# falcon-xu/DeViT

Hardware: AMD Instinct MI355X
Metric: images/sec distill_sub step (DeiT-B->dedeit, bs256, 224^2) (higher is better)
Workload: dtype bf16; 1 GPU; distill_sub step dedeit<-deit_base_distilled_patch16_224, num_division=4 (C=25), bs=256/GPU, 224x224, hard distillation, drop_path 0.1, AdamW+EMA; classes=25, global_batch=256, parallelism=dp1

## Files before the change

devit_amd/_lib.py:

```python
import ctypes as C
import os

import torch

_HERE = os.path.dirname(os.path.abspath(__file__))
LIB_PATH = os.environ.get("DEVIT_LIB_PATH") or os.path.join(_HERE, "libdevit_hip.so")

EPI_STORE_BF16, EPI_GELU_BF16, EPI_RESIDUAL_F32, EPI_PATCH_F32, EPI_DGELU_BF16, EPI_ATOMIC_F32, EPI_STORE_F32 = range(7)


class Epilogue(C.Structure):
    _fields_ = [("kind", C.c_int), ("out", C.c_void_p), ("ldc", C.c_int), ("bias", C.c_void_p),
                ("colscale", C.c_void_p), ("aux", C.c_void_p), ("aux_in", C.c_void_p), ("res", C.c_void_p),
                ("rowscale", C.c_void_p), ("rows_per_scale", C.c_int), ("pos", C.c_void_p),
                ("patch_tokens", C.c_int), ("extra_tokens", C.c_int), ("exact_gelu", C.c_int),
                ("out_batch_stride", C.c_longlong), ("m_valid", C.c_int), ("dtype16", C.c_int)]


class Operand(C.Structure):
    _fields_ = [("ptr", C.c_void_p), ("ld", C.c_int), ("kmajor", C.c_int), ("row_group", C.c_int),
                ("row_skip", C.c_int), ("batch_stride", C.c_longlong)]


ACT_LN1, ACT_MEAN1, ACT_RSTD1, ACT_QKV, ACT_ATTN_O, ACT_LSE, ACT_X1, ACT_ATT, ACT_LN2, ACT_MEAN2, ACT_RSTD2, ACT_H, ACT_H_PRE, \
    ACT_X2, ACT_COUNT = range(15)
BLK_SAVE, BLK_QKV_PAD, BLK_ATT = 1, 2, 4
BWD_DH_PRE, BWD_DLN2, BWD_DX1, BWD_G1, BWD_DATTN, BWD_DQKV, BWD_DLN1, BWD_LNWS, BWD_COUNT = range(9)


class BlockWeights(C.Structure):
    _fields_ = [(n, C.c_void_p) for n in ("n1w", "n1b", "qkv_b", "proj_b", "n2w", "n2b", "fc1_b", "fc2_b", "qkv_w16",
                                          "proj_w16", "fc1_w16", "fc2_w16", "head_gate", "neuron_gate")] + \
               [("num_heads", C.c_int), ("attn_width", C.c_int), ("hidden", C.c_int), ("dtype16", C.c_int), ("fc2_w16t", C.c_void_p)]


class BlockWgrads(C.Structure):
    _fields_ = [(n, C.c_void_p) for n in ("n1w", "n1b", "qkv_w", "qkv_b", "proj_w", "proj_b", "n2w", "n2b", "fc1_w",
                                          "fc1_b", "fc2_w", "fc2_b")]


class BlockActs(C.Structure):
    _fields_ = [("x", C.c_void_p), ("buf", C.c_void_p * 14), ("dp1", C.c_void_p), ("dp2", C.c_void_p), ("flags", C.c_int)]


class BlockBwdIO(C.Structure):
    _fields_ = [("dx", C.c_void_p), ("g2", C.c_void_p), ("dx_in", C.c_void_p), ("g_prev", C.c_void_p),
                ("prev_dp2", C.c_void_p), ("prev_fc2_b_grad", C.c_void_p), ("g2_bias_done", C.c_int),
                ("dqkv_add", C.c_void_p), ("ws", C.c_void_p * 8), ("lnws_bytes", C.c_size_t),
                ("defer_jobs", C.c_void_p), ("defer_count", C.c_void_p)]


class BlockDropout(C.Structure):
    _fields_ = [("seed", C.c_ulonglong), ("block", C.c_int), ("thr", C.c_uint), ("thr_attn", C.c_uint), ("scale_keep", C.c_float),
                ("scale_keep_attn", C.c_float), ("tmp", C.c_void_p)]


class IndexJob(C.Structure):
    _fields_ = [("src", C.c_void_p), ("dst", C.c_void_p), ("idx", C.c_void_p), ("rows", C.c_int), ("cols", C.c_int),
                ("src_ld", C.c_int), ("dst_ld", C.c_int), ("mode", C.c_int), ("elem", C.c_int)]


class WgradJob(C.Structure):
    _fields_ = [("a", C.c_void_p), ("lda", C.c_int), ("a_cols", C.c_int), ("b", C.c_void_p), ("ldb", C.c_int), ("out", C.c_void_p),
                ("ldc", C.c_int), ("transposed", C.c_int), ("a_colsum", C.c_void_p)]


class MixSample(C.Structure):
    _fields_ = [("mode", C.c_int), ("lam", C.c_float), ("y0", C.c_int), ("y1", C.c_int), ("x0", C.c_int), ("x1", C.c_int),
                ("reserved", C.c_int * 2)]


class OptChunk(C.Structure):
    _fields_ = [("first4", C.c_uint), ("count4", C.c_uint), ("segment", C.c_int), ("flags", C.c_int)]


OPT_CHUNK_GRANULES, OPT_CHUNK_NO_DECAY = 1024, 1

HAS_Y_BF16, HAS_Y_F32, HAS_DY_F32, HAS_DRES, HAS_DX, HAS_DX_BF16, HAS_DQKV_ADD = 1, 2, 4, 8, 16, 32, 64


class LaunchInfo(C.Structure):
    _fields_ = [("name", C.c_char_p)] + [(n, C.c_int) for n in ("a_kmajor", "b_kmajor", "kind", "M", "N", "K", "batch", "split_k", "rows",
                                                                "width", "q_rows", "has", "njobs", "a_cols")] + \
               [("flops", C.c_double), ("bytes", C.c_double)]


LAUNCH_OBSERVER = C.CFUNCTYPE(None, C.c_void_p, C.c_int, C.c_void_p, C.POINTER(LaunchInfo))

HSIC_BF16, HSIC_F16, HSIC_F32 = range(3)

DROP_POS, DROP_ATTN, DROP_PROJ, DROP_HIDDEN, DROP_FC2 = range(5)

ROUTE_TILE128, ROUTE_TILE256, ROUTE_FULL_ROW, ROUTE_GEMM4 = 1, 3, 4, 5

WGRAD_MAX_JOBS = 48
ABI_VERSION = 3
ABI_STRUCTS = {0: Epilogue, 1: Operand, 2: BlockWeights, 3: BlockWgrads, 4: BlockActs, 5: BlockBwdIO, 6: IndexJob, 7: WgradJob, 8: LaunchInfo, 9: BlockDropout,
               10: MixSample, 11: OptChunk}


class DevitError(RuntimeError):
    pass


_P, _I, _F, _Z, _LL = C.c_void_p, C.c_int, C.c_float, C.c_size_t, C.c_longlong
_U64, _U32 = C.c_ulonglong, C.c_uint

SIGNATURES = {
    "devit_version": (_I, []),
    "devit_last_error": (C.c_char_p, []),
    "devit_check_device": (_I, [_I]),
    "devit_abi_struct_size": (_Z, [_I]),
    "devit_set_launch_observer": (_I, [LAUNCH_OBSERVER, _P]),
    "devit_gemm_full_row_selected": (_I, [_I, _I, _I, _I]),
    "devit_wgrad_grouped": (_I, [C.POINTER(WgradJob), _I, _I, _I, _P]),
    "devit_gemm_bf16": (_I, [C.POINTER(Operand), C.POINTER(Operand), _I, _I, _I, _I, _I, C.POINTER(Epilogue), _P]),
    "devit_gemm_route": (_I, [C.POINTER(Operand), C.POINTER(Operand), _I, _I, _I, _I, _I, C.POINTER(Epilogue)]),
    "devit_set_reserved_cus": (_I, [_I]),
    "devit_get_reserved_cus": (_I, []),
    "devit_set_deterministic": (_I, [_I]),
    "devit_get_deterministic": (_I, []),
    "devit_det_workspace_bytes": (_Z, []),
    "devit_set_det_workspace": (_I, [_P, _Z]),
    "devit_layernorm_fwd": (_I, [_P, _I, _I, _I, _I, _P, _P, _F, _P, _P, _P, _P, _I, _P]),
    "devit_layernorm_bwd_workspace": (_Z, [_I, _I]),
    "devit_layernorm_bwd": (_I, [_P, _I, _P, _I, _I, _I, _I, _P, _P, _P, _P, _P, _P, _P, _I, _P, _P, _P, _I, _P, _Z, _P]),
    "devit_dgrad_layernorm_bwd_fused": (_I, [_I, _I, _I]),
    "devit_dgrad_layernorm_bwd": (_I, [_P, _P, _I, _I, _P, _P, _I, _I, _P, _P, _P, _P, _P, _P, _P, _I, _P, _P, _P, _I, _P, _Z, _P]),
    "devit_block_acts_sizes": (_I, [_I, _I, _I, _I, _I, _I, C.POINTER(C.c_size_t)]),
    "devit_block_bwd_sizes": (_I, [_I, _I, _I, _I, _I, C.POINTER(C.c_size_t)]),
    "devit_encoder_fwd": (_I, [_I, C.POINTER(BlockWeights), C.POINTER(BlockActs), _I, _I, _I, _F, _P]),
    "devit_block_bwd": (_I, [C.POINTER(BlockWeights), C.POINTER(BlockActs), C.POINTER(BlockWgrads), C.POINTER(BlockBwdIO),
                             _I, _I, _I, _F, _P]),
    "devit_encoder_fwd_drop": (_I, [_I, C.POINTER(BlockWeights), C.POINTER(BlockActs), C.POINTER(BlockDropout), _I, _I, _I, _F, _P]),
    "devit_block_bwd_drop": (_I, [C.POINTER(BlockWeights), C.POINTER(BlockActs), C.POINTER(BlockWgrads), C.POINTER(BlockBwdIO),
                                  C.POINTER(BlockDropout), _I, _I, _I, _F, _P]),
    "devit_attn_fwd": (_I, [_P, _P, _P, _P, _I, _I, _I, _I, _F, _I, _P]),
    "devit_attn_bwd": (_I, [_P, _P, _P, _P, _P, _P, _P, _I, _I, _I, _I, _F, _P]),
    "devit_attn_fwd_rows": (_I, [_P, _I, _P, _I, _P, _P, _P, _I, _I, _I, _I, _I, _F, _I, _P]),
    "devit_attn_bwd_rows": (_I, [_P, _I, _P, _I, _P, _P, _P, _P, _P, _I, _P, _I, _I, _I, _I, _I, _I, _F, _P]),
    "devit_dropout_mask": (_I, [_U64, _I, _I, _U32, _I, _I, _LL, _P, _P]),
    "devit_dropout_apply": (_I, [_P, _I, _I, _I, _I, _LL, _U64, _I, _I, _U32, _F, _P, _P]),
    "devit_dropout_residual": (_I, [_P, _P, _P, _P, _I, _I, _I, _U64, _I, _I, _U32, _F, _P]),
    "devit_attn_fwd_drop": (_I, [_P, _P, _P, _P, _I, _I, _I, _I, _F, _U64, _I, _U32, _F, _P]),
    "devit_attn_bwd_drop": (_I, [_P, _P, _P, _P, _P, _P, _P, _I, _I, _I, _I, _F, _U64, _I, _U32, _F, _P]),
    "devit_index_copy": (_I, [_P, _I, _I, _P]),
    "devit_hsic_target": (_I, [_P, _I, _I, _I, _P, _P, _Z, _P]),
    "devit_hsic_scores_workspace": (_Z, [_I, _I, _I]),
    "devit_hsic_scores": (_I, [_P, _I, _I, _I, _I, _I, _LL, _LL, _P, _P, _P, _P, _P, _Z, _P]),
    "devit_hsic_head_pairs": (_I, [_P, _I, _I, _P, _P]),
    "devit_im2row_bf16": (_I, [_P, _P, _I, _I, _I, _I, _I, _I, _P]),
    "devit_mix_im2row_bf16": (_I, [_P, _P, _P, _I, _I, C.c_double, _I, _I, _I, _I, _P]),
    "devit_mix_im2row_bf16_sized": (_I, [_P, _P, _P, _I, _I, C.c_double, _I, _I, _I, _I, _I, _I, _P]),
    "devit_mix_targets": (_I, [_P, _P, _I, _I, C.c_double, C.c_double, _P]),
    "devit_mix_im2row_table": (_I, [_P, _P, _P, _P, _P, _I, _P]),
    "devit_mix_im2row_table_sized": (_I, [_P, _P, _P, _P, _P, _I, _I, _I, _P]),
    "devit_mix_targets_table": (_I, [_P, _P, _P, _I, _I, C.c_double, _P]),
    "devit_embed_tokens": (_I, [_P, _P, _P, _P, _I, _I, _I, _P]),
    "devit_embed_bwd": (_I, [_P, _I, _I, _I, _I, _P, _P, _P, _P, _P, _I, _P]),
    "devit_cast_bf16": (_I, [_P, _P, _Z, _I, _P]),
    "devit_scale_cast_bf16": (_I, [_P, _P, _P, _I, _I, _I, _P]),
    "devit_colsum_workspace": (_Z, [_I, _I]),
    "devit_colsum_bf16": (_I, [_P, _I, _I, _I, _I, _I, _P, _I, _P, _Z, _P]),
    "devit_sgemm_small": (_I, [_P, _LL, _LL, _P, _LL, _LL, _P, _P, _I, _I, _I, _I, _F, _I, _P]),
    "devit_sumsq_workspace": (_Z, []),
    "devit_sumsq_f32": (_I, [_P, _Z, _P, _P, _Z, _P]),
    "devit_adamw_step": (_I, [_P, _P, _P, _P, _P, _P, _P, _P, _P, _Z, _F, _F, _F, _F, _F, _F, _F, _P]),
    "devit_sgd_step": (_I, [_P, _P, _P, _P, _P, _P, _P, _P, _Z, _F, _I, _F, _F, _F, _F, _P]),
    "devit_adam_l2_step": (_I, [_P, _P, _P, _P, _P, _P, _P, _P, _P, _Z, _F, _F, _F, _F, _F, _F, _F, _P]),
    "devit_lamb_workspace": (_Z, [_I, _I]),
    "devit_lamb_step": (_I, [_P, _P, _P, _P, _P, _P, _P, _P, _Z, _P, _I, _I, _I, _F, _F, _F, _F, _F, _F, _F, _P, _Z, _P]),
    "devit_cls_distill_loss": (_I, [_P, _P, _P, _P, _I, _I, _I, _F, _F, _P, _P, _P, _P]),
    "devit_token_mse": (_I, [_P, _P, _Z, _P, _P, _I, _P]),
    "devit_token_kldiv": (_I, [_P, _P, _Z, _I, _P, _P, _I, _P]),
    "devit_relation_stats": (_I, [_P, _P, _I, _I, _I, _I, _I, _P, _P, _P, _P, _P]),
    "devit_relation_grad": (_I, [_P, _P, _P, _P, _P, _I, _I, _I, _I, _I, _P, _I, _P]),
    "devit_add_scale_cast_bf16": (_I, [_P, _P, _P, _P, _I, _I, _I, _P]),
    "devit_hid_normalize": (_I, [_P, _P, _P, _I, _I, _I, _I, _I, _I, _F, _P]),
    "devit_hid_stats": (_I, [_P, _P, _I, _I, _I, _I, _P, _P, _P]),
    "devit_hid_grad": (_I, [_P, _P, _P, _I, _I, _I, _I, _P, _I, _P]),
    "devit_hid_normalize_bwd": (_I, [_P, _P, _P, _P, _I, _I, _I, _I, _I, _P]),
    "devit_gemm_f32": (_I, [_P, _LL, _LL, _LL, _LL, _P, _LL, _LL, _LL, _LL, _I, _I, _I, _I, _I, _LL, _LL, _I, _I, _F, _P, _I,
                            C.POINTER(Epilogue), _P]),
    "devit_softmax_rows_f32": (_I, [_P, _I, _I, _I, _F, _P, _P]),
    "devit_softmax_bwd_rows_f32": (_I, [_P, _P, _I, _I, _I, _F, _P]),
    "devit_im2row_f32": (_I, [_P, _P, _I, _P]),
    "devit_im2row_f32_sized": (_I, [_P, _P, _I, _I, _I, _P]),
    "devit_scale_rows_f32": (_I, [_P, _P, _P, _I, _I, _I, _P]),
    "devit_colsum_f32": (_I, [_P, _I, _I, _I, _P, _I, _P]),
    "devit_comm_unique_id": (_I, [_P]),
    "devit_comm_init": (_I, [_P, _I, _I, C.POINTER(C.c_void_p)]),
    "devit_comm_allreduce_f32": (_I, [_P, _P, _Z, _P]),
    "devit_comm_destroy": (_I, [_P]),
}

_lib = None
_checked_devices = set()


def load():
    global _lib
    if _lib is None:
        if not os.path.exists(LIB_PATH):
            raise DevitError(
                f"{LIB_PATH} not found: build it with `python -c 'import __graft_entry__ as g; g.build()'` "
                "(or devit_amd/csrc/build.sh).  devit_amd has no CPU / PyTorch fallback.")
        lib = C.CDLL(LIB_PATH)
        for name, (res, args) in SIGNATURES.items():
            fn = getattr(lib, name)
            fn.restype, fn.argtypes = res, args
        if lib.devit_version() != ABI_VERSION:
            raise DevitError(f"libdevit_hip.so ABI version {lib.devit_version()} != {ABI_VERSION} of this binding: rebuild (devit_amd/csrc/build.sh)")
        for which, cls in ABI_STRUCTS.items():
            if lib.devit_abi_struct_size(which) != C.sizeof(cls):
                raise DevitError(f"libdevit_hip.so: sizeof struct {which} = {lib.devit_abi_struct_size(which)}, the binding's {cls.__name__} has "
                                 f"{C.sizeof(cls)} bytes: header and binding disagree")
        _lib = lib
    return _lib


def require_device(t: torch.Tensor):
    if not t.is_cuda:
        raise DevitError("devit_amd ops run on MI355X (gfx950) only; got a %s tensor. There is no CPU fallback "
                         "(the CPU restatement lives in oracle/ and is test infrastructure)." % t.device)
    idx = t.device.index if t.device.index is not None else torch.cuda.current_device()
    if idx not in _checked_devices:
        call("devit_check_device", idx)
        _checked_devices.add(idx)


before_call = None


def call(name, *args):
    lib = load()
    if before_call is not None:
        before_call()
    rc = getattr(lib, name)(*args)
    if rc != 0:
        raise DevitError(f"{name} failed ({rc}): {lib.devit_last_error().decode()}")
    return rc


def stream_ptr():
    return C.c_void_p(torch.cuda.current_stream().cuda_stream)


def ptr(t):
    return None if t is None else C.c_void_p(t.data_ptr())
```

devit_amd/ops.py:

```python
import contextlib
import ctypes as C
import os

import numpy as np
import torch

from . import _lib as L
from ._lib import ptr, stream_ptr

BF16, F16, F32 = torch.bfloat16, torch.float16, torch.float32
ROW_TILE = 256


PROFILE = None
PROFILE_HBM = None
PROFILE_WGRAD = None


def gemm_template(a_kmajor, b_kmajor, kind, fused_ln_bwd=False):
    b_row = not b_kmajor or kind == L.EPI_RESIDUAL_F32
    return ("A_km" if a_kmajor else "A_row") + "/" + ("B_row" if b_row else "B_km") + ("+ln_bwd" if fused_ln_bwd else "")


def hbm_record(i):
# ... 1058 lines not shown


class HeadsFn(torch.autograd.Function):
    @staticmethod
    def forward(ctx, x, norm_w, norm_b, head_w, head_b, headd_w, headd_b, ntok, eps, grad_ready):
        L.require_device(x)
        x = x.contiguous()
        B, T, D = x.shape
        rows = B * ntok
        dev = x.device
        tok = torch.empty((B, ntok, D), dtype=F32, device=dev)
        mean = torch.empty(rows, dtype=F32, device=dev)
        rstd = torch.empty(rows, dtype=F32, device=dev)
        layernorm_fwd(x.view(B * T, D), rows, D, norm_w, norm_b, eps, y_f32=tok, mean=mean, rstd=rstd, in_group=ntok,
                      in_stride=T)
        outs = [tok]
        if head_w is not None:
            Cn = head_w.shape[0]
            lo = torch.empty((B, Cn), dtype=F32, device=dev)
            sgemm_small(tok, ntok * D, 1, head_w, D, 1, head_b, lo, Cn, B, Cn, D)
            outs.append(lo)
            if ntok == 2 and headd_w is not None:
                lk = torch.empty((B, Cn), dtype=F32, device=dev)
                sgemm_small(tok[:, 1], ntok * D, 1, headd_w, D, 1, headd_b, lk, Cn, B, Cn, D)
                outs.append(lk)
        ctx.save = (x, tok, mean, rstd)
        ctx.params = (norm_w, norm_b, head_w, head_b, headd_w, headd_b)
        ctx.meta = (B, T, D, ntok, eps, grad_ready)
        ctx.set_materialize_grads(False)
        return tuple(outs)

    @staticmethod
    def backward(ctx, dtok, dlo=None, dlk=None):
        x, tok, mean, rstd = ctx.save
        norm_w, norm_b, head_w, head_b, headd_w, headd_b = ctx.params
        B, T, D, ntok, eps, grad_ready = ctx.meta
        dev = x.device
        dt = torch.zeros((B, ntok, D), dtype=F32, device=dev) if dtok is None else dtok.contiguous().clone()
        for j, (dl, w, b) in enumerate(((dlo, head_w, head_b), (dlk, headd_w, headd_b))):
            if dl is None or w is None:
                continue
            dl = dl.contiguous()
            Cn = w.shape[0]
            sgemm_small(dl, Cn, 1, w, 1, D, None, dt[:, j], ntok * D, B, D, Cn, accumulate=True)
            sgemm_small(dl, 1, Cn, tok[:, j], 1, ntok * D, None, grad_buf(w), D, Cn, D, B, accumulate=True)
            ones = _ones1(dev)
            sgemm_small(dl, 1, Cn, ones, 0, 0, None, grad_buf(b), 1, Cn, 1, B, accumulate=True)
        dx = torch.zeros((B, T, D), dtype=F32, device=dev)
        layernorm_bwd(dt, True, x.view(B * T, D), B * ntok, D, mean, rstd, norm_w, None, dx.view(B * T, D), None, None,
                      0, grad_buf(norm_w), grad_buf(norm_b), in_group=ntok, in_stride=T)
        if grad_ready is not None:
            grad_ready([p for p in ctx.params if p is not None])
        return (dx,) + (None,) * 9


def _to_rows_bf16(x):
    B, N, D = x.shape
    M = B * N
    buf = rows_alloc(M, D, BF16, x.device)
    call("devit_scale_cast_bf16", ptr(x.contiguous().float()), ptr(buf), None, 0, M, D, stream_ptr())
    return buf


class MlpFn(torch.autograd.Function):
    @staticmethod
    def forward(ctx, x, module, w1, b1, w2, b2, w1_16, w2_16, gate, grad_enabled):
        L.require_device(x)
        B, N, D = x.shape
        M, dev, Hd, Do = B * N, x.device, w1.shape[0], w2.shape[0]
        xb = _to_rows_bf16(x)
        need = grad_enabled and (x.requires_grad or w1.requires_grad)
        h = rows_alloc(M, Hd, BF16, dev)
        h_pre = rows_alloc(M, Hd, BF16, dev) if need else None
        linear_fwd(xb, w1_16, b1, M, out=h, kind=L.EPI_GELU_BF16, colscale=gate, aux=h_pre, exact_gelu=0)
        y = torch.empty((B, N, Do), dtype=F32, device=dev)
        linear_fwd(h, w2_16, b2, M, out=y.view(M, Do), kind=L.EPI_STORE_F32)
        module.neuron_output = h[:M].view(B, N, Hd)
        ctx.s = (xb, h, h_pre, gate, w1, b1, w2, b2, w1_16, w2_16, (B, N, D))
        return y

    @staticmethod
    def backward(ctx, dy):
        xb, h, h_pre, gate, w1, b1, w2, b2, w1_16, w2_16, (B, N, D) = ctx.s
        M, dev, Hd = B * N, dy.device, w1.shape[0]
        g = _to_rows_bf16(dy)
        dh = rows_alloc(M, Hd, BF16, dev)
        linear_dgrad(g, w2_16, M, out=dh, kind=L.EPI_DGELU_BF16, colscale=gate, aux_in=h_pre)
        linear_wgrad(g, h, grad_buf(w2), grad_buf(b2), M)
        dx = torch.empty((B, N, D), dtype=F32, device=dev)
        linear_dgrad(dh, w1_16, M, out=dx.view(M, D), kind=L.EPI_STORE_F32)
        linear_wgrad(dh, xb, grad_buf(w1), grad_buf(b1), M)
        return (dx,) + (None,) * 9


class AttentionFn(torch.autograd.Function):
    @staticmethod
    def forward(ctx, x, module, wq, bq, wp, bp_, wq16, wp16, gate, grad_enabled):
        L.require_device(x)
        B, N, D = x.shape
        M, dev, H = B * N, x.device, module.num_heads
        xb = _to_rows_bf16(x)
        need = grad_enabled and (x.requires_grad or wq.requires_grad)
        qkv = rows_alloc(M, 3 * D, BF16, dev)
        linear_fwd(xb, wq16, bq, M, out=qkv)
        o = rows_alloc(M, D, BF16, dev)
        lse = torch.empty((B, H, N), dtype=F32, device=dev) if need else None
        call("devit_attn_fwd", ptr(qkv), ptr(o), ptr(lse), ptr(gate), B, N, H, D // H, (D // H) ** -0.5, 0, stream_ptr())
        y = torch.empty((B, N, D), dtype=F32, device=dev)
        linear_fwd(o, wp16, bp_, M, out=y.view(M, D), kind=L.EPI_STORE_F32)
        module.head_output = o[:M].view(B, N, H, D // H)
        ctx.s = (xb, qkv, o, lse, gate, wq, bq, wp, bp_, wq16, wp16, (B, N, D, H))
        return y, qkv

    @staticmethod
    def backward(ctx, dy, dqkv_in):
        xb, qkv, o, lse, gate, wq, bq, wp, bp_, wq16, wp16, (B, N, D, H) = ctx.s
        M, dev = B * N, dy.device
        g = _to_rows_bf16(dy)
        do = rows_alloc(M, D, BF16, dev)
        linear_dgrad(g, wp16, M, out=do)
        linear_wgrad(g, o, grad_buf(wp), grad_buf(bp_), M)
        dqkv = rows_alloc(M, 3 * D, BF16, dev)
        call("devit_attn_bwd", ptr(qkv), ptr(o), ptr(do), ptr(lse), ptr(gate),
             ptr(dqkv_in.contiguous()) if dqkv_in is not None else None, ptr(dqkv), B, N, H, D // H, (D // H) ** -0.5,
             stream_ptr())
        dx = torch.empty((B, N, D), dtype=F32, device=dev)
        linear_dgrad(dqkv, wq16, M, out=dx.view(M, D), kind=L.EPI_STORE_F32)
        linear_wgrad(dqkv, xb, grad_buf(wq), grad_buf(bq), M)
        return (dx,) + (None,) * 9


class ClsDistillLossFn(torch.autograd.Function):

    @staticmethod
    def forward(ctx, logits, logits_kd, teacher_logits, soft_targets, kind, alpha, tau):
        L.require_device(logits)
        logits, logits_kd = logits.contiguous().float(), logits_kd.contiguous().float()
        soft_targets = soft_targets.contiguous().float()
        tl = teacher_logits.contiguous().float() if teacher_logits is not None else None
        B, Cn = logits.shape
        loss3 = torch.empty(3, dtype=F32, device=logits.device)
        dlo, dlk = torch.empty_like(logits), torch.empty_like(logits_kd)
        call("devit_cls_distill_loss", ptr(logits), ptr(logits_kd), ptr(tl), ptr(soft_targets), B, Cn,
             {"none": 0, "soft": 1, "hard": 2}[kind], alpha, tau, ptr(loss3), ptr(dlo), ptr(dlk), stream_ptr())
        ctx.save_for_backward(dlo, dlk)
        return loss3[0]

    @staticmethod
    def backward(ctx, g):
        dlo, dlk = ctx.saved_tensors
        return dlo * g, dlk * g, None, None, None, None, None


class RelationLossFn(torch.autograd.Function):

    @staticmethod
    def forward(ctx, s_qkv, t_qkv, B, N, hd_s, hd_t):
        L.require_device(s_qkv)
        dev = s_qkv.device
        Ds, Dt = s_qkv.shape[1] // 3, t_qkv.shape[1] // 3
        assert s_qkv.shape[0] >= (B - 1) * N + 256 and t_qkv.shape[0] >= (B - 1) * N + 256, "packed qkv needs pad rows"
        losses = torch.empty(3, dtype=F32, device=dev)
        grams, stats = [], []
        for j in range(3):
            gt = torch.empty((B, 256, 256), dtype=F32, device=dev)
            gs = torch.empty((B, 256, 256), dtype=F32, device=dev)
            for buf, Dm, out in ((t_qkv, Dt, gt), (s_qkv, Ds, gs)):
                f = buf[:, j * Dm:]
                gemm(f, 3 * Dm, 0, f, 3 * Dm, 0, 256, 256, Dm, kind=L.EPI_STORE_F32, out=out, ldc=256, batch=B,
                     a_bs=N * 3 * Dm, b_bs=N * 3 * Dm, out_bs=256 * 256, dtype16=int(buf.dtype == F16))
            lse_t = torch.empty((B, N), dtype=F32, device=dev)
            lse_s = torch.empty((B, N), dtype=F32, device=dev)
            row_kl = torch.empty((B, N), dtype=F32, device=dev)
            call("devit_relation_stats", ptr(gt), ptr(gs), B, N, 256, hd_t, hd_s, ptr(lse_t), ptr(lse_s), ptr(row_kl),
                 ptr(losses[j:]), stream_ptr())
            grams.append((gt, gs))
            stats.append((lse_t, lse_s))
        ctx.grams, ctx.stats, ctx.s_qkv = grams, stats, s_qkv
        ctx.meta = (B, N, hd_s, hd_t, Ds)
        return losses

    @staticmethod
    def backward(ctx, g):
        B, N, hd_s, hd_t, Ds = ctx.meta
        s_qkv = ctx.s_qkv
        dev = s_qkv.device
        g = g.contiguous().float()
        d = torch.empty_like(s_qkv)
        S = torch.empty((B, 256, 256), dtype=BF16, device=dev)
        for j in range(3):
            gt, gs = ctx.grams[j]
            lse_t, lse_s = ctx.stats[j]
            call("devit_relation_grad", ptr(gt), ptr(gs), ptr(lse_t), ptr(lse_s), ptr(g[j:]), B, N, 256, hd_t, hd_s,
                 ptr(S), 0, stream_ptr())
            f = s_qkv[:, j * Ds:]
            gemm(S, 256, 0, f, 3 * Ds, 1, 256, Ds, 256, kind=L.EPI_STORE_BF16, out=d[:, j * Ds:], ldc=3 * Ds, batch=B,
                 a_bs=256 * 256, b_bs=N * 3 * Ds, out_bs=N * 3 * Ds, m_valid=N)
        ctx.grams = ctx.stats = None
        return d, None, None, None, None, None


HID_EPS = 1e-12


def hid_normalize(h, exact=False):
    L.require_device(h)
    if h.dim() != 3:
        raise L.DevitError(f"cal_hid_relation_loss: hidden states are [B, N, D], got {tuple(h.shape)}")
    B, N, D = h.shape
    h = h.contiguous().float()
    if h.data_ptr() % 16:
        h = h.clone()
    ld = (D + 127) // 128 * 128
    rows = pad_rows(B * N) + qkv_pad_rows(N)
    hn = torch.empty((rows, ld), dtype=F32 if exact else BF16, device=h.device)
    inv = torch.empty(B * N, dtype=F32, device=h.device)
    call("devit_hid_normalize", ptr(h), ptr(hn), ptr(inv), B, N, D, ld, rows, int(exact), HID_EPS, stream_ptr())
    return hn, inv


def hid_gram(hn, B, N, D, exact=False):
    ld = hn.shape[1]
    if exact:
        from .ops_f32 import sgemm
        g = torch.zeros((B, 256, 256), dtype=F32, device=hn.device)
        sgemm(hn, ld, 1, hn, ld, 1, N, N, D, out=g, ldc=256, batch=B, a_bo=N * ld, b_bo=N * ld, c_bo=65536)
        return g
    g = torch.empty((B, 256, 256), dtype=F32, device=hn.device)
    gemm(hn, ld, 0, hn, ld, 0, 256, 256, ld, kind=L.EPI_STORE_F32, out=g, ldc=256, batch=B, a_bs=N * ld, b_bs=N * ld, out_bs=65536)
    return g


def hid_stats(gs, gt, B, N, layers=1):
    row_sq = torch.empty(B * N, dtype=F32, device=gs.device)
    loss = torch.empty(1, dtype=F32, device=gs.device)
    call("devit_hid_stats", ptr(gs), ptr(gt), B, N, 256, layers, ptr(row_sq), ptr(loss), stream_ptr())
    return loss


def hid_grad(gs, gt, upstream, B, N, layers=1, exact=False):
    S = torch.empty((B, 256, 256), dtype=F32 if exact else BF16, device=gs.device)
    call("devit_hid_grad", ptr(gs), ptr(gt), ptr(upstream), B, N, 256, layers, ptr(S), int(exact), stream_ptr())
    return S


def hid_dhn(S, hn, B, N, D, exact=False):
    ld = hn.shape[1]
    if exact:
        from .ops_f32 import sgemm
        dhn = torch.zeros((B * N, ld), dtype=F32, device=hn.device)
        sgemm(S, 256, 1, hn, 1, ld, N, D, N, out=dhn, ldc=ld, batch=B, a_bo=65536, b_bo=N * ld, c_bo=N * ld)
        return dhn
    dhn = torch.empty((B * N, ld), dtype=F32, device=hn.device)
    gemm(S, 256, 0, hn, ld, 1, 256, ld, 256, kind=L.EPI_STORE_F32, out=dhn, ldc=ld, batch=B, a_bs=65536, b_bs=N * ld, out_bs=N * ld,
         m_valid=N)
    return dhn


def hid_normalize_bwd(hn, dhn, inv, B, N, D):
    dh = torch.empty((B, N, D), dtype=F32, device=hn.device)
    call("devit_hid_normalize_bwd", ptr(hn), ptr(dhn), ptr(inv), ptr(dh), B, N, D, hn.shape[1], int(hn.dtype == F32), stream_ptr())
    return dh


class HidRelationLossFn(torch.autograd.Function):

    @staticmethod
    def forward(ctx, s, t, layers, exact):
        B, N, Ds = s.shape
        if tuple(t.shape[:2]) != (B, N):
            raise L.DevitError(f"cal_hid_relation_loss: student {tuple(s.shape)} and teacher {tuple(t.shape)} differ in batch or tokens")
        hs, inv_s = hid_normalize(s, exact)
        ht, _ = hid_normalize(t, exact)
        gs, gt = hid_gram(hs, B, N, Ds, exact), hid_gram(ht, B, N, t.shape[2], exact)
        ctx.keep, ctx.meta = (hs, inv_s, gs, gt), (B, N, Ds, layers, exact)
        return hid_stats(gs, gt, B, N, layers)[0]

    @staticmethod
    def backward(ctx, g):
        hs, inv_s, gs, gt = ctx.keep
        B, N, Ds, layers, exact = ctx.meta
        ctx.keep = None
        S = hid_grad(gs, gt, g.contiguous().float(), B, N, layers, exact)
        return hid_normalize_bwd(hs, hid_dhn(S, hs, B, N, Ds, exact), inv_s, B, N, Ds), None, None, None
```

include/devit_hip.h:

```cpp
#ifndef DEVIT_HIP_H
#define DEVIT_HIP_H

#include <stddef.h>
#include <stdint.h>

#ifdef __cplusplus
extern "C" {
#endif

#define DEVIT_ABI_VERSION 3
#define DEVIT_API __attribute__((visibility("default")))

enum {
  DEVIT_OK = 0,
  DEVIT_ERR_SHAPE = -1,
  DEVIT_ERR_ARG = -2,
  DEVIT_ERR_LAUNCH = -3,
  DEVIT_ERR_DEVICE = -4
};

DEVIT_API int devit_version(void);
DEVIT_API const char* devit_last_error(void);
DEVIT_API int devit_check_device(int dev);
DEVIT_API size_t devit_abi_struct_size(int which);
// ... 110 lines not shown
                        float scale, unsigned long long seed, int block, unsigned thr, float scale_keep, void* stream);
DEVIT_API int devit_attn_bwd_drop(const void* qkv, const void* out, const void* dout, const float* lse, const float* head_gate,
                        const void* dqkv_add, void* dqkv, int B, int N, int H, int head_dim, float scale, unsigned long long seed,
                        int block, unsigned thr, float scale_keep, void* stream);

typedef struct {
  const float *n1w, *n1b, *qkv_b, *proj_b, *n2w, *n2b, *fc1_b, *fc2_b;
  const void *qkv_w16, *proj_w16, *fc1_w16, *fc2_w16;
  const float *head_gate, *neuron_gate;
  int num_heads, attn_width, hidden;
  int dtype16;
  const void* fc2_w16t;
} devit_block_weights;

typedef struct {
  float *n1w, *n1b, *qkv_w, *qkv_b, *proj_w, *proj_b, *n2w, *n2b, *fc1_w, *fc1_b, *fc2_w, *fc2_b;
} devit_block_wgrads;

enum { DEVIT_ACT_LN1 = 0, DEVIT_ACT_MEAN1, DEVIT_ACT_RSTD1, DEVIT_ACT_QKV, DEVIT_ACT_ATTN_O, DEVIT_ACT_LSE, DEVIT_ACT_X1,
       DEVIT_ACT_ATT, DEVIT_ACT_LN2, DEVIT_ACT_MEAN2, DEVIT_ACT_RSTD2, DEVIT_ACT_H, DEVIT_ACT_H_PRE, DEVIT_ACT_X2,
       DEVIT_ACT_COUNT };
enum { DEVIT_BLK_SAVE = 1, DEVIT_BLK_QKV_PAD = 2, DEVIT_BLK_ATT = 4 };

typedef struct {
  const float* x;
  void* buf[DEVIT_ACT_COUNT];
  const float *dp1, *dp2;
  int flags;
} devit_block_acts;

enum { DEVIT_BWD_DH_PRE = 0, DEVIT_BWD_DLN2, DEVIT_BWD_DX1, DEVIT_BWD_G1, DEVIT_BWD_DATTN, DEVIT_BWD_DQKV, DEVIT_BWD_DLN1,
       DEVIT_BWD_LNWS, DEVIT_BWD_COUNT };

typedef struct {
  const float* dx;
  const void* g2;
  float* dx_in;
  void* g_prev;
  const float* prev_dp2;
  float* prev_fc2_b_grad;
  int g2_bias_done;
  const void* dqkv_add;
  void* ws[DEVIT_BWD_COUNT];
  size_t lnws_bytes;
  devit_wgrad_job* defer_jobs;
  int* defer_count;
} devit_block_bwd_io;

DEVIT_API int devit_block_acts_sizes(int B, int N, int D, int attn_width, int hidden, int flags, size_t* sizes );
DEVIT_API int devit_block_bwd_sizes(int B, int N, int D, int attn_width, int hidden, size_t* sizes );
DEVIT_API int devit_encoder_fwd(int nblocks, const devit_block_weights* w, const devit_block_acts* acts, int B, int N, int D,
                      float eps, void* stream);
DEVIT_API int devit_block_bwd(const devit_block_weights* w, const devit_block_acts* acts, const devit_block_wgrads* grads,
                    const devit_block_bwd_io* io, int B, int N, int D, float eps, void* stream);

typedef struct {
  const void* src;
  void* dst;
  const int* idx;
  int rows, cols;
  int src_ld, dst_ld;
  int mode;
  int elem;
} devit_index_job;
DEVIT_API int devit_index_copy(const devit_index_job* jobs_device, int njobs, int blocks_per_job, void* stream);

enum { DEVIT_HSIC_BF16 = 0, DEVIT_HSIC_F16 = 1, DEVIT_HSIC_F32 = 2 };
DEVIT_API int devit_hsic_target(const float* y, int B, int C, int softmax, float* W, void* workspace, size_t workspace_bytes,
                      void* stream);
DEVIT_API size_t devit_hsic_scores_workspace(int B, int N, int units);
DEVIT_API int devit_hsic_scores(const void* X, int elem, int B, int N, int units, int group, long long batch_stride,
                      long long token_stride, const float* W, float* rel, float* act, float* kmix1, void* workspace,
                      size_t workspace_bytes, void* stream);
DEVIT_API int devit_hsic_head_pairs(const float* kmix1, int H, int B, float* red, void* stream);

DEVIT_API int devit_im2row_bf16(const float* img, void* rows, int B, int C, int H, int W, int patch, int dtype16, void* stream);
DEVIT_API int devit_mix_im2row_bf16(const float* img, void* rows , void* rows_f16 , int B, int mode,
                          double lam, int y0, int y1, int x0, int x1, void* stream);
DEVIT_API int devit_mix_im2row_bf16_sized(const float* img, void* rows , void* rows_f16 , int B, int mode,
                          double lam, int y0, int y1, int x0, int x1, int H, int W, void* stream);
DEVIT_API int devit_mix_targets(const long long* labels, float* targets, int B, int C, double lam, double smoothing, void* stream);
typedef struct {
  int mode;
  float lam;
  int y0, y1, x0, x1;
  int reserved[2];
} devit_mix_sample;
DEVIT_API int devit_mix_im2row_table(const float* img, void* rows , void* rows_f16 ,
                           float* img_out , const devit_mix_sample* table , int B,
                           void* stream);
DEVIT_API int devit_mix_im2row_table_sized(const float* img, void* rows , void* rows_f16 ,
                           float* img_out , const devit_mix_sample* table , int B,
                           int H, int W, void* stream);
DEVIT_API int devit_mix_targets_table(const long long* labels, float* targets, const devit_mix_sample* table, int B, int C,
                            double smoothing, void* stream);
DEVIT_API int devit_embed_tokens(const float* cls, const float* dist, const float* pos, float* x, int B, int T, int D,
                       void* stream);
DEVIT_API int devit_embed_bwd(const float* dx, int B, int T, int D, int ntok, float* dpos, float* dcls, float* ddist,
                    float* dbias, void* dx_bf16, int accumulate, void* stream);

DEVIT_API int devit_cast_bf16(const float* src, void* dst, size_t n, int dtype16, void* stream);

DEVIT_API int devit_scale_cast_bf16(const float* src, void* dst, const float* rowscale, int rows_per_scale, int M, int D,
                          void* stream);

DEVIT_API size_t devit_colsum_workspace(int M, int N);
DEVIT_API int devit_colsum_bf16(const void* y, int M, int N, int ld, int row_group, int row_skip, float* out, int accumulate,
                      void* workspace, size_t workspace_bytes, void* stream);

DEVIT_API int devit_sgemm_small(const float* A, long long sam, long long sak, const float* B, long long sbn, long long sbk,
                      const float* bias, float* C, int ldc, int M, int N, int K, float alpha, int accumulate,
                      void* stream);

DEVIT_API size_t devit_sumsq_workspace(void);
DEVIT_API int devit_sumsq_f32(const float* g, size_t n, float* out, void* workspace, size_t workspace_bytes, void* stream);
DEVIT_API int devit_adamw_step(float* p, const float* g, float* m, float* v, float* ema, void* p_bf16,
                     const unsigned char* no_decay4, const float* gnorm_sq, const float* dyn, size_t n, float beta1,
                     float beta2, float eps, float weight_decay, float max_norm, float ema_decay, float grad_scale,
                     void* stream);

typedef struct {
  unsigned first4;
  unsigned count4;
  int segment;
  int flags;
} devit_opt_chunk;
DEVIT_API int devit_sgd_step(float* p, const float* g, float* buf, float* ema, void* p_bf16, const unsigned char* no_decay4,
                   const float* gnorm_sq, const float* dyn, size_t n, float momentum, int nesterov, float weight_decay,
                   float max_norm, float ema_decay, float grad_scale, void* stream);
DEVIT_API int devit_adam_l2_step(float* p, const float* g, float* m, float* v, float* ema, void* p_bf16,
                       const unsigned char* no_decay4, const float* gnorm_sq, const float* dyn, size_t n, float beta1,
                       float beta2, float eps, float weight_decay, float max_norm, float ema_decay, float grad_scale,
                       void* stream);
DEVIT_API size_t devit_lamb_workspace(int nchunks, int nsegments);
DEVIT_API int devit_lamb_step(float* p, const float* g, float* m, float* v, float* ema, void* p_bf16, const float* gnorm_sq,
                    const float* dyn, size_t n, const devit_opt_chunk* chunks, int nchunks, int nsegments, int trust_clip,
                    float beta1, float beta2, float eps, float weight_decay, float max_norm, float ema_decay, float grad_scale,
                    void* workspace, size_t workspace_bytes, void* stream);

DEVIT_API int devit_cls_distill_loss(const float* logits, const float* logits_kd, const float* teacher_logits,
                           const float* soft_targets, int B, int C, int kind, float alpha, float tau, float* loss3,
                           float* dlogits, float* dlogits_kd, void* stream);

DEVIT_API int devit_token_mse(const float* a, const float* b, size_t n, float* loss, float* da, int accumulate, void* stream);

DEVIT_API int devit_token_kldiv(const float* s, const float* t, size_t n, int batch, float* loss, float* ds,
                                int accumulate, void* stream);

DEVIT_API int devit_relation_stats(const float* gram_t, const float* gram_s, int B, int N, int ldr, int head_dim_t,
                         int head_dim_s, float* lse_t, float* lse_s, float* row_kl, float* loss, void* stream);
DEVIT_API int devit_relation_grad(const float* gram_t, const float* gram_s, const float* lse_t, const float* lse_s,
                        const float* upstream, int B, int N, int ldr, int head_dim_t, int head_dim_s, void* S_out,
                        int out_is_f32, void* stream);

DEVIT_API int devit_add_scale_cast_bf16(float* dx, const float* add, void* g_bf16, const float* rowscale, int rows_per_scale, int M,
                              int D, void* stream);
DEVIT_API int devit_hid_normalize(const float* h, void* out, float* inv, int B, int N, int D, int ld, int rows_total, int out_is_f32,
                        float eps, void* stream);
DEVIT_API int devit_hid_stats(const float* gram_s, const float* gram_t, int B, int N, int ldr, int layers, float* row_sq, float* loss,
                    void* stream);
DEVIT_API int devit_hid_grad(const float* gram_s, const float* gram_t, const float* upstream, int B, int N, int ldr, int layers,
                   void* S_out, int out_is_f32, void* stream);
DEVIT_API int devit_hid_normalize_bwd(const void* hn, const float* dhn, const float* inv, float* dh, int B, int N, int D, int ld,
                            int hn_is_f32, void* stream);

DEVIT_API int devit_gemm_f32(const float* A, long long sam, long long sak, long long a_bs_outer, long long a_bs_inner,
                   const float* B, long long sbn, long long sbk, long long b_bs_outer, long long b_bs_inner, int M, int N,
                   int K, int batch, int batch_inner, long long c_bs_outer, long long c_bs_inner, int k_group, int k_skip,
                   float alpha, const float* batch_scale, int accumulate, const devit_epilogue* ep, void* stream);
DEVIT_API int devit_softmax_rows_f32(float* S, int rows, int ncols, int ld, float scale, float* lse, void* stream);
DEVIT_API int devit_softmax_bwd_rows_f32(const float* P, float* dP, int rows, int ncols, int ld, float scale, void* stream);
DEVIT_API int devit_im2row_f32(const float* img, float* rows, int B, void* stream);
DEVIT_API int devit_im2row_f32_sized(const float* img, float* rows, int B, int H, int W, void* stream);
DEVIT_API int devit_scale_rows_f32(const float* src, float* dst, const float* rowscale, int rows_per_scale, int M, int D,
                         void* stream);
DEVIT_API int devit_colsum_f32(const float* y, int M, int N, int ld, float* out, int accumulate, void* stream);

#define DEVIT_COMM_ID_BYTES 128
DEVIT_API int devit_comm_unique_id(void* id );
DEVIT_API int devit_comm_init(const void* id, int rank, int world, void** comm);
DEVIT_API int devit_comm_allreduce_f32(void* comm, float* buf, size_t count, void* stream);
DEVIT_API int devit_comm_destroy(void* comm);

typedef struct {
  unsigned long long seed;
  int block;
  unsigned thr, thr_attn;
  float scale_keep, scale_keep_attn;
  float* tmp;
} devit_block_dropout;
DEVIT_API int devit_encoder_fwd_drop(int nblocks, const devit_block_weights* w, const devit_block_acts* acts, const devit_block_dropout* drop,
                           int B, int N, int D, float eps, void* stream);
DEVIT_API int devit_block_bwd_drop(const devit_block_weights* w, const devit_block_acts* acts, const devit_block_wgrads* grads,
                         const devit_block_bwd_io* io, const devit_block_dropout* drop, int B, int N, int D, float eps, void* stream);

#ifdef __cplusplus
}
#endif
#endif
```

Measured before the change: 11610 images/sec.

## Fuse relation-loss gram, softmax stats and gradient into single HIP kernels

Adds a forward kernel that computes the teacher and student q/k/v gram matrices per sample in registers with MFMA. In the same kernel it computes log-sum-exp, row KL and the bf16 gradient matrix S, then reduces the loss in a small second kernel. A fused backward kernel multiplies S by the student features and applies the upstream scale in one pass. This removes the separate batched GEMMs, the fp32 256x256 gram tensors written to and read from HBM, and several launches per component, at the cost of shapes limited to N<=208 and heavy register use per 512-thread block. The new path is on by default and can be turned off with DEVIT_RELFUSE=0.

```diff
diff --git a/devit_amd/_lib.py b/devit_amd/_lib.py
--- a/devit_amd/_lib.py
+++ b/devit_amd/_lib.py
@@ -175,6 +175,8 @@
     "devit_token_kldiv": (_I, [_P, _P, _Z, _I, _P, _P, _I, _P]),
     "devit_relation_stats": (_I, [_P, _P, _I, _I, _I, _I, _I, _P, _P, _P, _P, _P]),
     "devit_relation_grad": (_I, [_P, _P, _P, _P, _P, _I, _I, _I, _I, _I, _P, _I, _P]),
+    "devit_relation_fused_fwd": (_I, [_P, _P, _I, _I, _I, _I, _I, _I, _I, _I, _I, _P, _P, _P, _P, _P, _P]),
+    "devit_relation_fused_bwd": (_I, [_P, _P, _P, _I, _I, _I, _I, _P, _I, _P]),
     "devit_add_scale_cast_bf16": (_I, [_P, _P, _P, _P, _I, _I, _I, _P]),
     "devit_hid_normalize": (_I, [_P, _P, _P, _I, _I, _I, _I, _I, _I, _F, _P]),
     "devit_hid_stats": (_I, [_P, _P, _I, _I, _I, _I, _P, _P, _P]),
diff --git a/devit_amd/csrc/relation.hip b/devit_amd/csrc/relation.hip
--- /dev/null
+++ b/devit_amd/csrc/relation.hip
@@ -0,0 +1,315 @@
+#include "devit_common.h"
+
+namespace {
+
+constexpr int RF_ROWS = 208;
+constexpr int RF_TILES = RF_ROWS / 16;
+constexpr int RF_SLD = 224;
+constexpr int RF_STRIDE = 144;
+constexpr int RF_STAGE = RF_ROWS * RF_STRIDE;
+constexpr int RF_SEGS = RF_ROWS * 8;
+
+struct RelFusedFwdArgs {
+  const __bf16* s; const __bf16* t;
+  float* lse_t; float* lse_s; float* row_kl;
+  __bf16* S;
+  int B, N, Ds, Dt, ld_s, ld_t;
+  float sc2_t, sc2_s;
+  float coef;
+};
+
+__device__ __forceinline__ float group16_max(float v) {
+#pragma unroll
+  for (int o = 8; o > 0; o >>= 1) v = fmaxf(v, __shfl_xor(v, o, 64));
+  return v;
+}
+__device__ __forceinline__ float group16_sum(float v) {
+#pragma unroll
+  for (int o = 8; o > 0; o >>= 1) v += __shfl_xor(v, o, 64);
+  return v;
+}
+
+template <bool F16>
+__device__ __forceinline__ void gram_accumulate(const __bf16* f, int ld, int D, int N, char* lds, int wave, int lane, bool two,
+                                                f32x4 (&acc)[2][RF_TILES]) {
+  const int tid = threadIdx.x;
+  const bf16x8 zero = {0, 0, 0, 0, 0, 0, 0, 0};
+  bf16x8 pf[4];
+  auto gload = [&](int c) {
+#pragma unroll
+    for (int u = 0; u < 4; ++u) {
+      const int sg = tid + u * 512, row = sg >> 3, piece = sg & 7;
+      pf[u] = (sg < RF_SEGS && row < N) ? *(const bf16x8*)(f + (size_t)row * ld + c * 64 + piece * 8) : zero;
+    }
+  };
+  auto lstore = [&](int stage) {
+#pragma unroll
+    for (int u = 0; u < 4; ++u) {
+      const int sg = tid + u * 512, row = sg >> 3, piece = sg & 7;
+      if (sg < RF_SEGS) *(bf16x8*)(lds + stage * RF_STAGE + row * RF_STRIDE + piece * 16) = pf[u];
+    }
+  };
+  const int nch = D / 64;
+  gload(0);
+  lstore(0);
+  __syncthreads();
+  const int frag = (lane & 15) * RF_STRIDE + (lane >> 4) * 16;
+  for (int c = 0; c < nch; ++c) {
+    if (c + 1 < nch) gload(c + 1);
+    const char* st = lds + (c & 1) * RF_STAGE + frag;
+#pragma unroll
+    for (int kk = 0; kk < 2; ++kk) {
+      const bf16x8 a0 = *(const bf16x8*)(st + wave * 16 * RF_STRIDE + kk * 64);
+      bf16x8 a1 = zero;
+      if (two) a1 = *(const bf16x8*)(st + (wave + 8) * 16 * RF_STRIDE + kk * 64);
+#pragma unroll
+      for (int J = 0; J < RF_TILES; ++J) {
+        const bf16x8 bj = *(const bf16x8*)(st + J * 16 * RF_STRIDE + kk * 64);
+        acc[0][J] = mfma16t<F16>(a0, bj, acc[0][J]);
+        if (two) acc[1][J] = mfma16t<F16>(a1, bj, acc[1][J]);
+      }
+    }
+    if (c + 1 < nch) lstore((c + 1) & 1);
+    __syncthreads();
+  }
+}
+
+template <bool TF16>
+__global__ __launch_bounds__(512) void rel_fused_fwd_kernel(const RelFusedFwdArgs a) {
+  __shared__ __attribute__((aligned(16))) char lds[2 * RF_STAGE];
+  __shared__ float lt_sh[RF_ROWS], ls_sh[RF_ROWS];
+  const int b = blockIdx.x, comp = blockIdx.y, N = a.N;
+  const int wave = __builtin_amdgcn_readfirstlane((int)(threadIdx.x >> 6)), lane = threadIdx.x & 63;
+  const bool two = wave + 8 < RF_TILES;
+  const int n = lane & 15, g = lane >> 4;
+  f32x4 at[2][RF_TILES], as[2][RF_TILES];
+#pragma unroll
+  for (int h = 0; h < 2; ++h)
+#pragma unroll
+    for (int J = 0; J < RF_TILES; ++J) at[h][J] = as[h][J] = (f32x4){0.f, 0.f, 0.f, 0.f};
+  gram_accumulate<TF16>(a.t + (size_t)b * N * a.ld_t + comp * a.Dt, a.ld_t, a.Dt, N, lds, wave, lane, two, at);
+  gram_accumulate<false>(a.s + (size_t)b * N * a.ld_s + comp * a.Ds, a.ld_s, a.Ds, N, lds, wave, lane, two, as);
+
+  const size_t stat0 = (size_t)comp * a.B * N + (size_t)b * N;
+#pragma unroll
+  for (int h = 0; h < 2; ++h) {
+    if (h == 0 || two) {
+#pragma unroll
+      for (int r = 0; r < 4; ++r) {
+        const int i = (wave + 8 * h) * 16 + 4 * g + r;
+        float mt = -INFINITY, ms = -INFINITY;
+#pragma unroll
+        for (int J = 0; J < RF_TILES; ++J) {
+          const bool valid = J * 16 + n < N;
+          at[h][J][r] = valid ? at[h][J][r] * a.sc2_t : -INFINITY;
+          as[h][J][r] = valid ? as[h][J][r] * a.sc2_s : -INFINITY;
+          mt = fmaxf(mt, at[h][J][r]);
+          ms = fmaxf(ms, as[h][J][r]);
+        }
+        mt = group16_max(mt);
+        ms = group16_max(ms);
+        float st = 0.f, ss = 0.f;
+#pragma unroll
+        for (int J = 0; J < RF_TILES; ++J) {
+          st += __builtin_amdgcn_exp2f(at[h][J][r] - mt);
+          ss += __builtin_amdgcn_exp2f(as[h][J][r] - ms);
+        }
+        const float lt = mt + log2f(group16_sum(st)), ls = ms + log2f(group16_sum(ss));
+        float kl = 0.f;
+#pragma unroll
+        for (int J = 0; J < RF_TILES; ++J)
+          if (J * 16 + n < N) {
+            const float a_t = at[h][J][r] - lt, a_s = as[h][J][r] - ls;
+            kl += __builtin_amdgcn_exp2f(a_t) * (a_t - a_s);
+          }
+        kl = group16_sum(kl) * (1.0f / LOG2E);
+        if (n == 0) {
+          lt_sh[i] = lt;
+          ls_sh[i] = ls;
+          if (i < N) {
+            a.lse_t[stat0 + i] = lt * (1.0f / LOG2E);
+            a.lse_s[stat0 + i] = ls * (1.0f / LOG2E);
+            a.row_kl[stat0 + i] = kl;
+          }
+        }
+      }
+    }
+  }
+  __syncthreads();
+
+  __bf16* const Sb = a.S + ((size_t)comp * a.B + b) * RF_ROWS * RF_SLD;
+#pragma unroll
+  for (int h = 0; h < 2; ++h) {
+    if (h == 0 || two) {
+      const int i0 = (wave + 8 * h) * 16 + 4 * g;
+      float lti[4], lsi[4];
+#pragma unroll
+      for (int r = 0; r < 4; ++r) {
+        lti[r] = lt_sh[i0 + r];
+        lsi[r] = ls_sh[i0 + r];
+      }
+#pragma unroll
+      for (int J = 0; J < RF_TILES; ++J) {
+        const int j = J * 16 + n;
+        const float ltj = lt_sh[j], lsj = ls_sh[j];
+        f32x4 v;
+#pragma unroll
+        for (int r = 0; r < 4; ++r) {
+          const float t = at[h][J][r], s = as[h][J][r];
+          const float e = (__builtin_amdgcn_exp2f(s - lsi[r]) + __builtin_amdgcn_exp2f(s - lsj) - __builtin_amdgcn_exp2f(t - lti[r]) -
+                           __builtin_amdgcn_exp2f(t - ltj)) * a.coef;
+          v[r] = (i0 + r < N && j < N) ? e : 0.f;
+        }
+        *(bf16x4*)(Sb + (size_t)j * RF_SLD + i0) = (bf16x4){f2bf(v[0]), f2bf(v[1]), f2bf(v[2]), f2bf(v[3])};
+      }
+      *(bf16x4*)(Sb + (size_t)((wave + 8 * h) * 16 + (lane >> 2)) * RF_SLD + RF_ROWS + (lane & 3) * 4) = (bf16x4){0, 0, 0, 0};
+    }
+  }
+}
+
+__global__ __launch_bounds__(1024) void rel_fused_reduce_kernel(const float* row_kl, int n, float inv_b, float* loss) {
+  __shared__ float red[16];
+  const float* src = row_kl + (size_t)blockIdx.x * n;
+  float p[8] = {0.f, 0.f, 0.f, 0.f, 0.f, 0.f, 0.f, 0.f};
+  for (int i0 = threadIdx.x; i0 < n; i0 += 8 * 1024) {
+#pragma unroll
+    for (int u = 0; u < 8; ++u) {
+      const int i = i0 + u * 1024;
+      p[u] += i < n ? src[i] : 0.f;
+    }
+  }
+  float s = ((p[0] + p[1]) + (p[2] + p[3])) + ((p[4] + p[5]) + (p[6] + p[7]));
+  s = wave_sum(s);
+  if ((threadIdx.x & 63) == 0) red[threadIdx.x >> 6] = s;
+  __syncthreads();
+  if (threadIdx.x == 0) {
+    float t = 0.f;
+#pragma unroll
+    for (int w = 0; w < 16; ++w) t += red[w];
+    loss[blockIdx.x] = t * inv_b;
+  }
+}
+
+struct RelFusedBwdArgs {
+  const __bf16* S;
+  const __bf16* s;
+  const float* upstream;
+  __bf16* d;
+  int B, N, Ds, ld_s, ld_d;
+};
+constexpr int RB_STAGE = RF_SLD * RF_STRIDE;
+constexpr int RB_SEGS = RF_SLD * 8;
+__global__ __launch_bounds__(512, 4) void rel_fused_bwd_kernel(const RelFusedBwdArgs a) {
+  __shared__ __attribute__((aligned(16))) char lds[2 * RB_STAGE];
+  const int b = blockIdx.x, comp = blockIdx.y, N = a.N, nch = a.Ds / 64;
+  const int wave = __builtin_amdgcn_readfirstlane((int)(threadIdx.x >> 6)), lane = threadIdx.x & 63, tid = threadIdx.x;
+  const bool two = wave + 8 < RF_TILES;
+  const int n = lane & 15, g = lane >> 4;
+  const __bf16* const f = a.s + (size_t)b * N * a.ld_s + comp * a.Ds;
+  const bf16x8 zero = {0, 0, 0, 0, 0, 0, 0, 0};
+  const unsigned foff = (unsigned)(tid >> 3) * (unsigned)a.ld_s + (tid & 7) * 8;
+  bf16x8 pf[4];
+  auto gload = [&](int c) {
+#pragma unroll
+    for (int u = 0; u < 4; ++u) {
+      const int row = (tid >> 3) + u * 64;
+      pf[u] = (row < RF_SLD && row < N) ? *(const bf16x8*)((f + c * 64 + (size_t)u * 64 * a.ld_s) + foff) : zero;
+    }
+  };
+  auto lstore = [&](int stage) {
+#pragma unroll
+    for (int u = 0; u < 4; ++u) {
+      const int sg = tid + u * 512, row = sg >> 3, piece = sg & 7;
+      if (sg < RB_SEGS) *(bf16x8*)(lds + stage * RB_STAGE + row * RF_STRIDE + piece * 16) = pf[u];
+    }
+  };
+  gload(0);
+  const __bf16* const Sl = a.S + (((size_t)comp * a.B + b) * RF_ROWS + wave * 16 + n) * RF_SLD + g * 8;
+  bf16x8 sf[2][7];
+#pragma unroll
+  for (int ks = 0; ks < 7; ++ks) {
+    sf[0][ks] = *(const bf16x8*)(Sl + ks * 32);
+    sf[1][ks] = two ? *(const bf16x8*)(Sl + (size_t)128 * RF_SLD + ks * 32) : zero;
+  }
+  lstore(0);
+  __syncthreads();
+  const float up = a.upstream[comp];
+  const int trd = (8 * g + (n >> 2)) * RF_STRIDE + (n & 3) * 8;
+  for (int c = 0; c < nch; ++c) {
+    if (c + 1 < nch) gload(c + 1);
+    const char* const st = lds + (c & 1) * RB_STAGE + trd;
+    f32x4 acc[2][4];
+#pragma unroll
+    for (int h = 0; h < 2; ++h)
+#pragma unroll
+      for (int ct = 0; ct < 4; ++ct) acc[h][ct] = (f32x4){0.f, 0.f, 0.f, 0.f};
+#pragma unroll
+    for (int ks = 0; ks < 7; ++ks) {
+#pragma unroll
+      for (int ct = 0; ct < 4; ++ct) {
+        const char* p = st + ks * 32 * RF_STRIDE + ct * 32;
+        const bf16x8 ff = cat8(lds_tr_read(p), lds_tr_read(p + 4 * RF_STRIDE));
+        acc[0][ct] = mfma16(ff, sf[0][ks], acc[0][ct]);
+        if (two) acc[1][ct] = mfma16(ff, sf[1][ks], acc[1][ct]);
+      }
+    }
+#pragma unroll
+    for (int h = 0; h < 2; ++h) {
+      const int i = (wave + 8 * h) * 16 + n;
+      if ((h == 0 || two) && i < N) {
+        __bf16* const o = a.d + ((size_t)b * N + i) * a.ld_d + comp * a.Ds + c * 64 + 4 * g;
+#pragma unroll
+        for (int ct = 0; ct < 4; ++ct) {
+          const f32x4 v = acc[h][ct];
+          *(bf16x4*)(o + ct * 16) = (bf16x4){f2bf(v[0] * up), f2bf(v[1] * up), f2bf(v[2] * up), f2bf(v[3] * up)};
+        }
+      }
+    }
+    if (c + 1 < nch) lstore((c + 1) & 1);
+    __syncthreads();
+  }
+}
+
+bool rel_fused_shape_ok(int B, int N, int D, int ld) {
+  return B > 0 && N > 0 && N <= RF_ROWS && D > 0 && D <= 1024 && D % 64 == 0 && ld >= 3 * D && ld % 8 == 0;
+}
+
+}
+
+extern "C" int devit_relation_fused_fwd(const void* s_qkv, const void* t_qkv, int B, int N, int Ds, int Dt, int ld_s, int ld_t,
+                                        int head_dim_t, int head_dim_s, int teacher_f16, float* lse_t, float* lse_s, float* row_kl,
+                                        void* S_out, float* loss3, void* stream) {
+  DEVIT_CHECK(s_qkv && t_qkv && lse_t && lse_s && row_kl && S_out && loss3, DEVIT_ERR_ARG, "devit_relation_fused_fwd: null pointer");
+  DEVIT_CHECK(((uintptr_t)s_qkv | (uintptr_t)t_qkv | (uintptr_t)S_out) % 16 == 0, DEVIT_ERR_ARG,
+              "devit_relation_fused_fwd: the qkv buffers and S must be 16-byte aligned");
+  DEVIT_CHECK(rel_fused_shape_ok(B, N, Ds, ld_s) && rel_fused_shape_ok(B, N, Dt, ld_t) && head_dim_t > 0 && head_dim_s > 0 &&
+                  (long long)B * N < (1ll << 31) / 3,
+              DEVIT_ERR_SHAPE,
+              "devit_relation_fused_fwd: B=%d N=%d Ds=%d Dt=%d ld_s=%d ld_t=%d: N <= 208, widths multiples of 64 up to 1024, row strides multiples "
+              "of 8 and >= 3 widths",
+              B, N, Ds, Dt, ld_s, ld_t);
+  RelFusedFwdArgs a{(const __bf16*)s_qkv, (const __bf16*)t_qkv, lse_t, lse_s, row_kl, (__bf16*)S_out, B, N, Ds, Dt, ld_s, ld_t,
+                    (float)(1.4426950408889634 / sqrt((double)head_dim_t)), (float)(1.4426950408889634 / sqrt((double)head_dim_s)),
+                    1.0f / ((float)B * sqrtf((float)head_dim_s))};
+  if (teacher_f16) hipLaunchKernelGGL(rel_fused_fwd_kernel<true>, dim3(B, 3), dim3(512), 0, (hipStream_t)stream, a);
+  else hipLaunchKernelGGL(rel_fused_fwd_kernel<false>, dim3(B, 3), dim3(512), 0, (hipStream_t)stream, a);
+  DEVIT_LAUNCH_CHECK();
+  hipLaunchKernelGGL(rel_fused_reduce_kernel, dim3(3), dim3(1024), 0, (hipStream_t)stream, (const float*)row_kl, B * N, 1.0f / (float)B, loss3);
+  DEVIT_LAUNCH_CHECK();
+  return DEVIT_OK;
+}
+
+extern "C" int devit_relation_fused_bwd(const void* S, const void* s_qkv, const float* upstream3, int B, int N, int Ds, int ld_s, void* d,
+                                        int ld_d, void* stream) {
+  DEVIT_CHECK(S && s_qkv && upstream3 && d, DEVIT_ERR_ARG, "devit_relation_fused_bwd: null pointer");
+  DEVIT_CHECK(((uintptr_t)S | (uintptr_t)s_qkv) % 16 == 0 && (uintptr_t)d % 8 == 0, DEVIT_ERR_ARG,
+              "devit_relation_fused_bwd: S and the qkv buffer must be 16-byte aligned, d 8-byte aligned");
+  DEVIT_CHECK(rel_fused_shape_ok(B, N, Ds, ld_s) && ld_d >= 3 * Ds && ld_d % 4 == 0, DEVIT_ERR_SHAPE,
+              "devit_relation_fused_bwd: B=%d N=%d Ds=%d ld_s=%d ld_d=%d: N <= 208, Ds a multiple of 64 up to 1024, ld_s a multiple of 8, ld_d of 4, "
+              "both >= 3 Ds",
+              B, N, Ds, ld_s, ld_d);
+  RelFusedBwdArgs a{(const __bf16*)S, (const __bf16*)s_qkv, upstream3, (__bf16*)d, B, N, Ds, ld_s, ld_d};
+  hipLaunchKernelGGL(rel_fused_bwd_kernel, dim3(B, 3), dim3(512), 0, (hipStream_t)stream, a);
+  DEVIT_LAUNCH_CHECK();
+  return DEVIT_OK;
+}
diff --git a/devit_amd/ops.py b/devit_amd/ops.py
--- a/devit_amd/ops.py
+++ b/devit_amd/ops.py
@@ -1234,6 +1234,16 @@
         return dlo * g, dlk * g, None, None, None, None, None
 
 
+def relation_fused_selected(s_qkv, t_qkv, B, N):
+    if os.environ.get("DEVIT_RELFUSE", "") == "0":
+        return False
+    Ds, Dt = s_qkv.shape[1] // 3, t_qkv.shape[1] // 3
+    return (s_qkv.dtype == BF16 and t_qkv.dtype in (BF16, F16) and 0 < N <= 208 and B > 0
+            and all(0 < D <= 1024 and D % 64 == 0 for D in (Ds, Dt))
+            and all(b.dim() == 2 and b.shape[1] == 3 * D and b.stride(1) == 1 and b.stride(0) % 8 == 0 and b.shape[0] >= B * N
+                    and b.data_ptr() % 16 == 0 for b, D in ((s_qkv, Ds), (t_qkv, Dt))))
+
+
 class RelationLossFn(torch.autograd.Function):
 
     @staticmethod
@@ -1241,6 +1251,16 @@
         L.require_device(s_qkv)
         dev = s_qkv.device
         Ds, Dt = s_qkv.shape[1] // 3, t_qkv.shape[1] // 3
+        ctx.fused = relation_fused_selected(s_qkv, t_qkv, B, N)
+        if ctx.fused:
+            losses = torch.empty(3, dtype=F32, device=dev)
+            stats = torch.empty((3, 3, B * N), dtype=F32, device=dev)
+            S = torch.empty((3, B, 208, 224), dtype=BF16, device=dev)
+            call("devit_relation_fused_fwd", ptr(s_qkv), ptr(t_qkv), B, N, Ds, Dt, s_qkv.stride(0), t_qkv.stride(0), hd_t, hd_s,
+                 int(t_qkv.dtype == F16), ptr(stats[0]), ptr(stats[1]), ptr(stats[2]), ptr(S), ptr(losses), stream_ptr())
+            ctx.S, ctx.s_qkv = S, s_qkv
+            ctx.meta = (B, N, hd_s, hd_t, Ds)
+            return losses
         assert s_qkv.shape[0] >= (B - 1) * N + 256 and t_qkv.shape[0] >= (B - 1) * N + 256, "packed qkv needs pad rows"
         losses = torch.empty(3, dtype=F32, device=dev)
         grams, stats = [], []
@@ -1269,6 +1289,10 @@
         dev = s_qkv.device
         g = g.contiguous().float()
         d = torch.empty_like(s_qkv)
+        if ctx.fused:
+            call("devit_relation_fused_bwd", ptr(ctx.S), ptr(s_qkv), ptr(g), B, N, Ds, s_qkv.stride(0), ptr(d), d.stride(0), stream_ptr())
+            ctx.S = None
+            return d, None, None, None, None, None
         S = torch.empty((B, 256, 256), dtype=BF16, device=dev)
         for j in range(3):
             gt, gs = ctx.grams[j]
diff --git a/include/devit_hip.h b/include/devit_hip.h
--- a/include/devit_hip.h
+++ b/include/devit_hip.h
@@ -286,6 +286,11 @@
 DEVIT_API int devit_relation_grad(const float* gram_t, const float* gram_s, const float* lse_t, const float* lse_s,
                         const float* upstream, int B, int N, int ldr, int head_dim_t, int head_dim_s, void* S_out,
                         int out_is_f32, void* stream);
+DEVIT_API int devit_relation_fused_fwd(const void* s_qkv, const void* t_qkv, int B, int N, int Ds, int Dt, int ld_s, int ld_t,
+                             int head_dim_t, int head_dim_s, int teacher_f16, float* lse_t, float* lse_s, float* row_kl,
+                             void* S_out, float* loss3, void* stream);
+DEVIT_API int devit_relation_fused_bwd(const void* S, const void* s_qkv, const float* upstream3, int B, int N, int Ds, int ld_s, void* d,
+                             int ld_d, void* stream);
 
 DEVIT_API int devit_add_scale_cast_bf16(float* dx, const float* add, void* g_bf16, const float* rowscale, int rows_per_scale, int M,
                               int D, void* stream);
```

Result: faster. 11780 images/sec, median of 6 (+1.4%).
